# FutureAGI/Xenoverse

Measured on AMD Instinct MI355X. Metric: env-steps/sec (whole node), anymdp |S|=64 |A|=8, 65k envs/GPU, higher is better.
Workload: dtype f64

## Files before the change

### xenoverse_amd/csrc/anymdp.hip

```cpp
#include "anymdp_cutline.h"
#include "philox.h"
#include "xv_common.h"
#include "xv_pipe.h"

#include <cstddef>
#include <cstdlib>
#include <cstring>
#include <mutex>

#define XV_ANYMDP_BLK 7
#define XV_ANYMDP_MAX_CHAINS 16
#ifndef XV_ANYMDP_NT_OUT
#define XV_ANYMDP_NT_OUT 1
#endif

struct AnyMDPArgs {
  const uint4* lines;
  const int32_t* state_map;
  const uint64_t* term_mask;
  const double* s0_cdf;
  const int32_t* s0_ids;
  const int32_t* max_steps;
  const int32_t* env_task;
  const double2* rs_a;
// ... 1406 lines not shown
      __syncthreads();
      if (own) Qs[tid] = qn;
    } else {
      for (int k = tid; k < SA; k += blockDim.x) {
        const int s = k / A, a = k - s * A;
        double qn = 0.0;
        if (!((tm[s >> 6] >> (s & 63)) & 1ull)) {
          const uint32_t r = ((uint32_t)t * S + s) * A + a;
          double prev = 0.0, acc = 0.0, e_r = 0.0;
          for (int j = 0; j < S; ++j) {
            const uint4 e = *anymdp_entry_ptr(P, r, j);
            const double c = xv_u2d(e.x, e.y), p = c - prev;
            prev = c;
            e_r = fma(p, (double)__uint_as_float(e.z), e_r);
            acc = fma(p, Vs[j], acc);
          }
          qn = fma(gamma, acc, e_r);
        }
        const double q = Qs[k];
        d2 += (qn - q) * (qn - q);
        Qs[SA + ((S + 63) & ~63) + blockDim.x + k] = qn;
      }
      __syncthreads();
      for (int k = tid; k < SA; k += blockDim.x) Qs[k] = Qs[SA + ((S + 63) & ~63) + blockDim.x + k];
    }
    red[tid] = d2;
    __syncthreads();
    for (int w = blockDim.x >> 1; w > 0; w >>= 1) {
      if (tid < w) red[tid] += red[tid + w];
      __syncthreads();
    }
    const double diff = sqrt(red[0] / (double)SA);
    __syncthreads();
    if (diff <= tol) { ++it; break; }
  }
  if (q_out) for (int k = tid; k < SA; k += blockDim.x) q_out[(size_t)t * SA + k] = Qs[k];
  if (greedy_out) {
    for (int j = tid; j < S; j += blockDim.x) {
      int best = 0;
      double v = Qs[j * A];
      for (int a = 1; a < A; ++a) if (Qs[j * A + a] > v) { v = Qs[j * A + a]; best = a; }
      greedy_out[(size_t)t * S + j] = (uint8_t)best;
    }
  }
  if (iters_out && tid == 0) iters_out[t] = it;
}

static inline void anymdp_bind_rng(xv_anymdp* h, uint64_t ticks, bool advance = true) {
  h->a.seed = h->eng->seed;
  h->a.gid_base = h->eng->env_id_base;
  const XvTickBind b = xv_engine_bind_tick(h->eng, ticks, advance);
  h->a.tick = b.tick;
  h->a.tick_dev = b.tick_dev;
}

#define XV_ANYMDP_AUTO_FALLBACKS_CACHED 0.2
#define XV_ANYMDP_AUTO_FALLBACKS_HBM 0.5
static inline double anymdp_auto_fallback_limit(const xv_anymdp* h) {
  const double fence_bytes = (double)h->a.n_task * h->a.S * h->a.A * 128.0;
  return fence_bytes <= 128.0 * 1048576.0 ? XV_ANYMDP_AUTO_FALLBACKS_CACHED : XV_ANYMDP_AUTO_FALLBACKS_HBM;
}
static inline int anymdp_effective_search(const xv_anymdp* h) {
  if (h->search == XV_ANYMDP_SEARCH_BINARY || !h->fast) return XV_ANYMDP_SEARCH_BINARY;
  if (h->a.bucket != nullptr &&
      (h->search == XV_ANYMDP_SEARCH_BUCKET || (h->search == XV_ANYMDP_SEARCH_AUTO && h->census.auto_uses_bucket)))
    return XV_ANYMDP_SEARCH_BUCKET;
  return XV_ANYMDP_SEARCH_FENCE;
}

#ifndef XV_KERNELS_ONLY
static void anymdp_pipe_clear(xv_anymdp* h) {
  h->overlap = 0; h->pipe_failed = false; h->pipe_used_last = false; h->side = nullptr; h->side_for = nullptr;
  memset(&h->gate, 0, sizeof(h->gate));
  h->side_ev[0] = h->side_ev[1] = nullptr;
  h->pgraph[0] = h->pgraph[1] = nullptr; h->pgraph_exec[0] = h->pgraph_exec[1] = nullptr;
  h->tgraph[0] = h->tgraph[1] = nullptr; h->tgraph_exec[0] = h->tgraph_exec[1] = nullptr;
  memset(&h->tpipe_key, 0, sizeof(h->tpipe_key));
  h->d_ptick = nullptr; h->ptick_value = 0; h->ptick_valid = false;
  h->d_snap = nullptr; h->d_snap_w = nullptr; h->fell_seen = 0;
  h->backoff.fell_known = 0; h->backoff.left = 0; h->backoff.len = 32;
  h->backoff_mixed.fell_known = 0; h->backoff_mixed.left = 0; h->backoff_mixed.len = 0;
  memset(&h->pipe_key, 0, sizeof(h->pipe_key));
}
static XvPipeLanes anymdp_pipe_lanes(xv_anymdp* h, bool tokens, int D = 0) {
  XvPipeLanes L;
  L.D = D; L.main = h->eng->stream; L.side_for = &h->side_for; L.fork = &h->side_ev[0];
  L.side[0] = &h->side; L.join[0] = &h->side_ev[1];
  for (int q = 0; q < 2; ++q) {
    L.graph[q] = tokens ? &h->tgraph[q] : &h->pgraph[q];
    L.exec[q] = tokens ? &h->tgraph_exec[q] : &h->pgraph_exec[q];
  }
  for (int i = 0; i < XV_PIPE_DEPTH_MAX - 2; ++i) {
    XvPipeDeepLanes& X = h->gate.deep;
    L.side[1 + i] = &X.side[i]; L.join[1 + i] = &X.join[i]; L.graph[2 + i] = &X.graph[i]; L.exec[2 + i] = &X.exec[i];
  }
  return L;
}
static void anymdp_pipe_drop_graphs(xv_anymdp* h) {
  xv_pipe_drop_set(anymdp_pipe_lanes(h, false));
  xv_pipe_drop_set(anymdp_pipe_lanes(h, true));
  memset(&h->pipe_key, 0, sizeof(h->pipe_key));
  memset(&h->tpipe_key, 0, sizeof(h->tpipe_key));
  h->gate.unroll[0] = h->gate.unroll[1] = 0;
  h->gate.depth = 0;
  h->ptick_valid = false;
}
static void anymdp_pipe_release(xv_anymdp* h) {
  anymdp_pipe_drop_graphs(h);
  xv_pipe_release_streams(anymdp_pipe_lanes(h, false));
  if (h->d_ptick) (void)hipFree(h->d_ptick);
  if (h->d_snap) (void)hipFree(h->d_snap);
  if (h->d_snap_w) (void)hipFree(h->d_snap_w);
  xv_pipe_gate_destroy(&h->gate);
  anymdp_pipe_clear(h);
}

extern "C" int xv_anymdp_create(xv_engine* e, int n_env, int n_task, int S, int A, int s0_max,
                                void* rows, const int32_t* state_map, const uint64_t* term_mask,
                                const double* s0_cdf, const int32_t* s0_ids, const int32_t* max_steps,
                                const int32_t* env_task, xv_anymdp** out) {
  XV_CHECK_ARG(out != nullptr);
  *out = nullptr;
  XV_CHECK_ARG(e != nullptr);
  XV_CHECK_ARG(n_env > 0 && n_task > 0);
  XV_CHECK_ARG(S >= 2 && S <= 512 && A >= 2 && A <= 64 && s0_max >= 1 && s0_max <= 256);
  XV_CHECK_ARG(rows && state_map && term_mask && s0_cdf && s0_ids && max_steps && env_task);
  const int NB0 = (S + XV_ANYMDP_BLK - 1) / XV_ANYMDP_BLK, G = (NB0 + 15) / 16;
  const int NB = (NB0 + G - 1) / G * G, RL = 1 + NB;
  XV_CHECK_ARG((uint64_t)n_task * S * A * RL < 0xFFFFFFFFull);
  XV_HIP(hipSetDevice(e->device));
  xv_anymdp* h = new (std::nothrow) xv_anymdp();
  if (!h) {
    xv_set_error("xv_anymdp_create: out of host memory");
    return XV_ERR_NOMEM;
  }
  h->eng = e;
  h->search = XV_ANYMDP_SEARCH_AUTO;
  h->fast = false;
  h->obs_cdf = nullptr; h->n_obs = 0; h->d_obs = 0; h->d_act = 0; h->obs_bucket = nullptr;
  h->max_obs = -1;
  memset(&h->census, 0, sizeof(h->census));
  h->graph_mode = 2; h->graph_failed = false; h->graph = nullptr; h->graph_exec = nullptr;
  h->d_tick = nullptr; h->d_tick_value = 0; h->d_tick_valid = false;
  memset(&h->graph_key, 0, sizeof(h->graph_key));
  h->parent = nullptr; h->view_lo = 0; h->n_views = 0; h->chain_ev = nullptr;
  h->cgraph = nullptr; h->cgraph_exec = nullptr;
  memset(&h->cgraph_key, 0, sizeof(h->cgraph_key));
  anymdp_pipe_clear(h);
  AnyMDPArgs& a = h->a;
  memset(&a, 0, sizeof(a));
  a.lines = (const uint4*)rows; a.state_map = state_map; a.term_mask = term_mask;
  a.s0_cdf = s0_cdf; a.s0_ids = s0_ids; a.max_steps = max_steps; a.env_task = env_task;
  a.n_env = n_env; a.n_task = n_task; a.S = S; a.A = A; a.s0_max = s0_max; a.words = (S + 63) / 64;
  a.NB = NB; a.RL = RL; a.G = G;
  a.err = e->d_err;
  a.seed = e->seed; a.gid_base = e->env_id_base; a.tick = 0;

  bool fast = (G <= 5 && s0_max <= 4);
  auto device_max = [&](const int32_t* p, size_t n, int* out_max) -> hipError_t {
    int* d_max = nullptr;
    hipError_t r = hipMalloc(&d_max, sizeof(int));
    if (r == hipSuccess) r = hipMemsetAsync(d_max, 0, sizeof(int), e->stream);
    if (r == hipSuccess) {
      hipLaunchKernelGGL(anymdp_max_obs_kernel, dim3((unsigned)((n + 255) / 256)), dim3(256), 0, e->stream, p, n, d_max);
      r = hipMemcpyAsync(out_max, d_max, sizeof(int), hipMemcpyDeviceToHost, e->stream);
    }
    if (r == hipSuccess) r = hipStreamSynchronize(e->stream);
    if (d_max) (void)hipFree(d_max);
    return r;
  };
  {
    int h_max = 0;
    hipError_t r = hipSuccess;
    if (fast) {
      r = device_max(state_map, (size_t)n_task * S, &h_max);
      fast = r == hipSuccess && h_max < 65536;
      if (r == hipSuccess) h->max_obs = h_max;
    }
    if (fast) {
      r = device_max(max_steps, (size_t)n_task, &h_max);
      fast = r == hipSuccess && h_max < (1 << 27);
    }
    if (r != hipSuccess) {
// ... 572 lines not shown
```

### xenoverse_amd/csrc/anymdp_many.h

```cpp
#pragma once

struct AnyMDPRings {
  size_t stride;
  const int32_t* actions; int32_t* obs; float* reward; float* reward_gt; uint8_t* terminated; uint8_t* truncated; int32_t* final_obs;
  AnyMDPStepIO slot(int j) const {
    const size_t o = (size_t)j * stride;
    return anymdp_io(actions + o, obs + o, reward + o, reward_gt + o, terminated + o, truncated + o, final_obs ? final_obs + o : nullptr);
  }
  AnyMDPRings shifted(size_t lo) const {
    return AnyMDPRings{stride, actions + lo, obs + lo, reward + lo, reward_gt + lo, terminated + lo, truncated + lo,
                       final_obs ? final_obs + lo : nullptr};
  }
};

struct AnyMDPTokRings {
  const int32_t* actions; int32_t* obs; float* reward; float* reward_gt; uint8_t* terminated; uint8_t* truncated; int32_t* final_obs;
  AnyMDPTokIO slot(const xv_anymdp* h, int j) const {
    const size_t o = (size_t)j * (size_t)h->a.n_env, da = (size_t)h->d_act, dob = (size_t)h->d_obs;
    return anymdp_tok_io(actions + o * da, obs + o * dob, reward + o, reward_gt + o, terminated + o, truncated + o,
                         final_obs ? final_obs + o * dob : nullptr);
  }
};

template <class R> static void anymdp_ring_pointers(const R& r, const void** p) {
// ... 99 lines not shown
  h->d_tick_valid = false;
}

template <class Ensure>
static bool anymdp_many_prepare(xv_anymdp* h, int n_steps, int period, bool wanted, bool sticky, Ensure&& ensure) {
  h->graph_used_last = false;
  if (n_steps / period <= 0 || period <= 1 || h->graph_failed || !wanted) return false;
  bool ok = ensure();
  if (ok && !(h->d_tick_valid && h->d_tick_value == h->eng->tick)) {
    hipLaunchKernelGGL(anymdp_set_tick_kernel, dim3(1), dim3(1), 0, h->eng->stream, h->d_tick, h->eng->tick);
    ok = hipGetLastError() == hipSuccess;
    if (ok) { h->d_tick_value = h->eng->tick; h->d_tick_valid = true; }
  }
  if (!ok) anymdp_many_failed(h, sticky);
  return ok;
}

static bool anymdp_many_cycle(xv_anymdp* h, hipGraphExec_t exec, int period, bool sticky) {
  if (hipGraphLaunch(exec, h->eng->stream) != hipSuccess) {
    anymdp_many_failed(h, sticky);
    return false;
  }
  h->eng->tick += (uint64_t)period;
  h->d_tick_value = h->eng->tick;
  h->d_tick_valid = true;
  h->graph_used_last = true;
  return true;
}

static int anymdp_many_plain(xv_anymdp* h, int k, int period, const AnyMDPRings& R, int mode) {
  anymdp_bind_rng(h, 1);
  return anymdp_launch_step<false>(h, R.slot(k % period), 1, mode);
}

#define XV_ANYMDP_PIPE_GRAPH_MIN 64
static bool anymdp_pipe_setup(xv_anymdp* h, int* D) {
  const XvPipeLanes L = anymdp_pipe_lanes(h, false);
  if (xv_pipe_streams_stale(L)) anymdp_pipe_drop_graphs(h);
  const int got = xv_pipe_ensure_streams(L, *D);
  if (got == 0) return false;
  if (got < *D) (void)hipGetLastError();
  *D = got;
  if (!h->d_ptick && hipMalloc(&h->d_ptick, XV_PIPE_DEPTH_MAX * sizeof(uint64_t)) != hipSuccess) return false;
  if (!h->gate.d_seen && !xv_pipe_gate_create(&h->gate)) return false;
  if (!h->d_snap && hipMalloc(&h->d_snap, (size_t)h->a.n_env * sizeof(uint2)) != hipSuccess) { h->d_snap = nullptr; return false; }
  if (!h->d_snap_w) {
    if (hipMalloc(&h->d_snap_w, 4 * sizeof(uint32_t)) != hipSuccess) { h->d_snap_w = nullptr; return false; }
    if (hipMemsetAsync(h->d_snap_w, 0, 4 * sizeof(uint32_t), h->eng->stream) != hipSuccess) return false;
  }
  return true;
}
static bool anymdp_launch_replay(xv_anymdp* h, int eff, const AnyMDPStepIO& io, int period, int cycles, int mode, uint64_t t0) {
  AnyMDPArgs a = h->a;
  a.seed = h->eng->seed; a.gid_base = h->eng->env_id_base; a.tick = t0; a.tick_dev = nullptr;
  const dim3 grid(xv_div_up(h->a.n_env, 256)), block(256);
  uint32_t* h_fell = h->gate.d_issued + 1;
  anymdp_select_variant(h->a.G, anymdp_variant_bk(h, eff), -1, [&](auto v) {
    using V = decltype(v);
    if constexpr (V::g != 0)
      hipLaunchKernelGGL((anymdp_replay_kernel<V::g, V::bk>), grid, block, 0, h->eng->stream, a, io, period, cycles, mode,
                         (const uint2*)h->d_snap, h->d_snap_w, h->a.err, h_fell);
  });
  return hipGetLastError() == hipSuccess;
}

template <class K, class Node>
static int anymdp_pipe_graph_set(xv_anymdp* h, bool tokens, int D, int period, int cycles, const K& want, K* key, Node&& node,
                                 bool buildable = true) {
  const hipGraphExec_t* exec = tokens ? h->tgraph_exec : h->pgraph_exec;
  const bool same = exec[0] && exec[1] && anymdp_key_same(want, *key);
  const int have = (same && h->gate.depth == D) ? h->gate.unroll[tokens] : 0;
  const int U = xv_pipe_pick_unroll(period, cycles, have, D);
  if (U == 0 || U == have) return U;
  anymdp_pipe_drop_graphs(h);
  if (!buildable || !xv_pipe_build_set(anymdp_pipe_lanes(h, tokens, D), &h->gate, U, period, reinterpret_cast<void*>(&anymdp_pipe_head_kernel),
                                       h->d_ptick, h->a.err, node))
    return -1;
  h->gate.depth = D;
  anymdp_key_store(key, want);
  h->gate.unroll[tokens] = U;
  return U;
}

static int anymdp_pipe_graphs(xv_anymdp* h, int D, int period, int cycles, const AnyMDPRings& R, int mode) {
  const int eff = anymdp_effective_search(h);
  decltype(h->pipe_key) want;
  memset(&want, 0, sizeof want);
  want.period = period; want.mode = mode; want.search = eff; want.stride = R.stride;
  anymdp_ring_pointers(R, want.ptrs);
  want.bucket = (const void*)h->a.bucket; want.seed = h->eng->seed; want.gid_base = h->eng->env_id_base;
  void* fn = anymdp_graph_step_fn(h, eff, mode, true);
  AnyMDPStepNode sn;
  return anymdp_pipe_graph_set(h, false, D, period, cycles, want, &h->pipe_key, [&](int g, int slot, int q, hipKernelNodeParams* np) {
    sn.fill(np, h, fn, h->d_ptick + q, g, slot, R, mode);
  }, fn != nullptr);
}

static __global__ __launch_bounds__(256) void anymdp_pipe_open_kernel(uint2* sr, int n, uint32_t tag, uint64_t* tick_words, int n_words,
                                                                      uint64_t tick_base, uint2* snap, uint32_t* snap_w, uint32_t* err,
                                                                      int bad_tag_env, int repairable) {
  const int i = blockIdx.x * blockDim.x + threadIdx.x;
  if (i < n) {
    uint2 r = sr[i];
    r.x &= (1u << XV_ANYMDP_SR_TAG_SHIFT) - 1u;
    snap[i] = r;
    r.x |= (i == bad_tag_env ? ((tag + 77u) & 0x3FFFu) : tag) << XV_ANYMDP_SR_TAG_SHIFT;
    sr[i] = r;
  }
  if (i < n_words) tick_words[i] = tick_base;
  if (i == 0 && repairable) { const uint32_t e = *err; snap_w[0] = e; snap_w[1] = 0u; snap_w[2] = 0u; *err = e & ~(uint32_t)XV_DEVERR_HANDOFF; }
}

template <class Graphs, class Replay>
static int anymdp_pipe_call(xv_anymdp* h, int n_steps, int ring_period, int min_steps, const void* fn, bool tokens, int32_t* obs,
                            size_t n_obs, int* issued, Graphs&& graphs, Replay&& replay) {
  *issued = 0;
  int D = xv_pipe_preflight(n_steps, ring_period, min_steps, &h->backoff, &h->gate, fn, 256, (size_t)xv_div_up(h->a.n_env, 256),
                            h->eng->device, h->eng->stream);
  if (D == 0) return XV_OK;
  const int U = anymdp_pipe_setup(h, &D) ? graphs(D, n_steps / ring_period) : -1;
  if (U < 0) {
    (void)hipGetLastError();
    h->pipe_failed = true;
    return XV_OK;
  }
  if (U == 0) return XV_OK;
  const int cycles = n_steps / ring_period / U, period = ring_period * U;
  hipStream_t st = h->eng->stream;
  const int test_bad_tag = getenv("XV_PIPE_TEST_BAD_TAG") ? atoi(getenv("XV_PIPE_TEST_BAD_TAG")) : 0;
  const int test_fail = getenv("XV_PIPE_TEST_FAIL") ? atoi(getenv("XV_PIPE_TEST_FAIL")) : 0;
  h->fell_seen = __atomic_load_n(h->gate.h_issued + 1, __ATOMIC_ACQUIRE);
  const uint64_t t0 = h->eng->tick;
  hipLaunchKernelGGL(anymdp_pipe_open_kernel, dim3(xv_div_up(h->a.n_env, 256)), dim3(256), 0, st, h->a.sr, h->a.n_env,
                     XV_ANYMDP_SR_TAG(t0), h->d_ptick, XV_PIPE_DEPTH_MAX, t0 - (uint64_t)period, h->d_snap, h->d_snap_w,
                     h->a.err, test_bad_tag ? 0 : -1, 1);
  const XvPipeLanes L = anymdp_pipe_lanes(h, tokens, h->gate.depth);
  h->ptick_valid = false;
  if (hipGetLastError() != hipSuccess || !xv_pipe_fork(L)) {
    (void)hipGetLastError();
    h->pipe_failed = true;
    return XV_OK;
  }
  const XvPipeIssued r = xv_pipe_issue(L, &h->gate, cycles);
  const int k = r.cycles * period;
  h->eng->tick = t0 + (uint64_t)k;
  if (r.cycles < cycles) { (void)hipGetLastError(); h->pipe_failed = true; }
  *issued = k;
  if (r.broken || !r.joined) {
    (void)hipGetLastError();
    h->pipe_failed = true;
    xv_set_error("xv_anymdp_step_many: an overlapped ring cycle could be issued only in part; the envs' states are undefined");
    return XV_ERR_HIP;
  }
  if (k > 0) {
    if (test_fail)
      hipLaunchKernelGGL(anymdp_test_fail_kernel, dim3(xv_div_up(h->a.n_env, 256)), dim3(256), 0, st, h->a.sr, h->a.n_env, h->a.err, obs, n_obs);
    if (!replay(k, t0)) {
      (void)hipGetLastError();
      h->pipe_failed = true;
    }
    h->ptick_value = h->eng->tick; h->ptick_valid = true; h->graph_used_last = true; h->pipe_used_last = true;
  }
  return XV_OK;
}

static int anymdp_pipe_run(xv_anymdp* h, int n_steps, int period, const AnyMDPRings& R, int mode, int* issued) {
  static const int min_steps = getenv("XV_ANYMDP_PIPE_MIN_STEPS") ? atoi(getenv("XV_ANYMDP_PIPE_MIN_STEPS")) : XV_ANYMDP_PIPE_GRAPH_MIN;
  const int eff = anymdp_effective_search(h);
  return anymdp_pipe_call(h, n_steps, period, min_steps, anymdp_graph_step_fn(h, eff, mode, true), false, R.obs, (size_t)period * (size_t)h->a.n_env,
                          issued, [&](int D, int cycles) { return anymdp_pipe_graphs(h, D, period, cycles, R, mode); },
                          [&](int k, uint64_t t0) { return anymdp_launch_replay(h, eff, R.slot(0), period, k / period, mode, t0); });
}

extern "C" int xv_anymdp_set_step_many_overlap(xv_anymdp* h, int on) {
  XV_CHECK_ARG(h != nullptr && (on == 0 || on == 1));
  const int dev = h->eng->device;
  XV_CHECK_ARG(dev >= 0 && dev < 64);
  if (on) {
    if (h->parent != nullptr) {
      xv_set_error("xv_anymdp_set_step_many_overlap: not on a view (overlap the parent's step_many instead)");
      return XV_ERR_UNSUPPORTED;
    }
    if (!xv_device_overlap_acquire(dev, h)) {
      xv_set_error("xv_anymdp_set_step_many_overlap: another handle on device %d has the overlap on; one at a time", dev);
      return XV_ERR_UNSUPPORTED;
    }
    h->pipe_failed = false;
    xv_pipe_backoff_reset(&h->backoff, &h->gate);
    h->backoff_mixed.len = 0;
  } else {
    xv_device_overlap_release(dev, h);
  }
  h->overlap = on;
  return XV_OK;
}

extern "C" int xv_anymdp_step_many_overlap_state(xv_anymdp* h) {
  if (!h) return 0;
  if (h->pipe_failed) return -1;
  if (h->overlap && h->pipe_used_last && h->gate.h_issued &&
      __atomic_load_n(h->gate.h_issued + 1, __ATOMIC_ACQUIRE) != h->fell_seen)
    return -2;
  return (h->overlap && h->pipe_used_last) ? 1 : 0;
}

extern "C" int xv_anymdp_step_many(xv_anymdp* h, int n_steps, int period, const int32_t* actions,
                                   int32_t* obs, float* reward, float* reward_gt, uint8_t* terminated,
                                   uint8_t* truncated, int32_t* final_obs, int autoreset_mode) {
  XV_CHECK_ARG(h && n_steps > 0 && period > 0);
  XV_CHECK_ARG(actions && obs && reward && reward_gt && terminated && truncated);
  XV_CHECK_ARG(autoreset_mode >= 0 && autoreset_mode <= 2);
  const AnyMDPRings R{(size_t)h->a.n_env, actions, obs, reward, reward_gt, terminated, truncated, final_obs};
  int k = 0;
  const int cycles = n_steps / period;
  h->pipe_used_last = false;
  if (h->overlap && h->graph_mode != 0 && !h->eng->dev_tick && !h->pipe_failed &&
      anymdp_effective_search(h) != XV_ANYMDP_SEARCH_BINARY) {
    XV_HIP(hipSetDevice(h->eng->device));
    h->graph_used_last = false;
    const int rc = anymdp_pipe_run(h, n_steps, period, R, autoreset_mode, &k);
    if (rc != XV_OK) return rc;
  }
  if (k == 0 && anymdp_many_prepare(h, n_steps, period, anymdp_graph_wanted(h, n_steps), true,
                                    [&] { return anymdp_ensure_graph(h, period, R, autoreset_mode); }))
    for (int c = 0; c < cycles && anymdp_many_cycle(h, h->graph_exec, period, true); ++c) k += period;
  for (; k < n_steps; ++k) {
    const int rc = anymdp_many_plain(h, k, period, R, autoreset_mode);
    if (rc != XV_OK) return rc;
  }
  return XV_OK;
}

static bool anymdp_ensure_chain_graph(xv_anymdp* p, xv_anymdp* const* views, int n_views, int period, const AnyMDPRings& R, int mode) {
  const int eff = anymdp_effective_search(p);
  decltype(p->cgraph_key) want;
  memset(&want, 0, sizeof want);
  want.period = period; want.mode = mode; want.search = eff; want.n_views = n_views;
  anymdp_ring_pointers(R, want.ptrs);
  want.bucket = (const void*)p->a.bucket;
  for (int v = 0; v < n_views; ++v) want.views[v] = (const void*)views[v];
  if (p->cgraph_exec && anymdp_key_same(want, p->cgraph_key)) return true;
  anymdp_drop_chain_graph(p);
  if (!p->d_tick && hipMalloc(&p->d_tick, sizeof(uint64_t)) != hipSuccess) return false;
  if (hipGraphCreate(&p->cgraph, 0) != hipSuccess) return false;
  hipGraphNode_t tails[XV_ANYMDP_MAX_CHAINS];
  for (int v = 0; v < n_views; ++v) {
    tails[v] = nullptr;
    if (!anymdp_add_chain(views[v], p->cgraph, &tails[v], p->d_tick, eff, period, R.shifted((size_t)views[v]->view_lo), mode)) return false;
  }
  if (!anymdp_add_tick_node(p->cgraph, tails, n_views, p->d_tick, period)) return false;
  if (hipGraphInstantiate(&p->cgraph_exec, p->cgraph, nullptr, nullptr, 0) != hipSuccess) { p->cgraph_exec = nullptr; return false; }
  anymdp_key_store(&p->cgraph_key, want);
  return true;
// ... 31 lines not shown
  }
  int k = 0;
  if (how == 1) {
    if (anymdp_many_prepare(p, n_steps, period, p->graph_mode != 0, false,
                            [&] { return anymdp_ensure_chain_graph(p, views, n_views, period, R, autoreset_mode); }))
      for (int c = 0; c < cycles && anymdp_many_cycle(p, p->cgraph_exec, period, false); ++c) k += period;
    for (; k < n_steps; ++k) {
      const int rc = anymdp_many_plain(p, k, period, R, autoreset_mode);
      if (rc != XV_OK) return rc;
    }
    for (int v = 0; v < n_views; ++v) views[v]->eng->tick = t0 + (uint64_t)n_steps;
    return XV_OK;
  }
  if (!p->chain_ev) XV_HIP(hipEventCreateWithFlags(&p->chain_ev, hipEventDisableTiming));
  XV_HIP(hipEventRecord(p->chain_ev, p->eng->stream));
  bool all_graph = true;
  for (int v = 0; v < n_views; ++v) {
    xv_anymdp* h = views[v];
    if (h->eng->stream != p->eng->stream) XV_HIP(hipStreamWaitEvent(h->eng->stream, p->chain_ev, 0));
    all_graph = anymdp_many_prepare(h, n_steps, period, h->graph_mode != 0, true,
                                    [&] { return anymdp_ensure_graph(h, period, Rv(v), autoreset_mode); }) && all_graph;
  }
  int rc = XV_OK;
  if (all_graph) {
    for (int c = 0; c < cycles && all_graph; ++c) {
      for (int v = 0; v < n_views; ++v) all_graph = anymdp_many_cycle(views[v], views[v]->graph_exec, period, true) && all_graph;
      if (all_graph) k += period;
    }
    p->graph_used_last = k > 0;
  }
  for (int v = 0; v < n_views; ++v) k = (int)(views[v]->eng->tick - t0) > k ? (int)(views[v]->eng->tick - t0) : k;
  for (int v = 0; v < n_views && rc == XV_OK; ++v)
    for (int kk = (int)(views[v]->eng->tick - t0); kk < k && rc == XV_OK; ++kk)
      rc = anymdp_many_plain(views[v], kk, period, Rv(v), autoreset_mode);
  for (; k < n_steps && rc == XV_OK; ++k)
    for (int v = 0; v < n_views && rc == XV_OK; ++v) rc = anymdp_many_plain(views[v], k, period, Rv(v), autoreset_mode);
  for (int v = 0; v < n_views; ++v) {
    xv_anymdp* h = views[v];
    if (h->eng->stream == p->eng->stream) continue;
    if (!h->chain_ev && hipEventCreateWithFlags(&h->chain_ev, hipEventDisableTiming) != hipSuccess) { rc = rc == XV_OK ? XV_ERR_HIP : rc; continue; }
    if (hipEventRecord(h->chain_ev, h->eng->stream) != hipSuccess ||
        hipStreamWaitEvent(p->eng->stream, h->chain_ev, 0) != hipSuccess)
      rc = rc == XV_OK ? XV_ERR_HIP : rc;
  }
  if (rc == XV_ERR_HIP) xv_set_error("xv_anymdp_step_many_chains: joining the chains failed: %s", hipGetErrorString(hipGetLastError()));
  if (rc == XV_OK) p->eng->tick = t0 + (uint64_t)n_steps;
  return rc;
}

static int anymdp_tok_pipe_graphs(xv_anymdp* h, int D, int period, int cycles, const AnyMDPTokRings& R, int mode) {
  decltype(h->tpipe_key) want;
  memset(&want, 0, sizeof want);
  want.period = period; want.mode = mode; want.fmt = h->a.bfmt; want.d_obs = h->d_obs; want.d_act = h->d_act;
  anymdp_ring_pointers(R, want.ptrs);
  want.bucket = (const void*)h->a.bucket; want.obs_bucket = (const void*)h->obs_bucket;
  want.seed = h->eng->seed; want.gid_base = h->eng->env_id_base;
  void* fn = anymdp_tok_hand_fn(h);
  AnyMDPArgs a;
  AnyMDPTokArgs KA{h->obs_cdf, h->n_obs, h->d_obs, h->d_act, h->obs_bucket};
  AnyMDPTokIO io;
  int md = mode;
  void* params[] = {&a, &KA, &io, &md};
  return anymdp_pipe_graph_set(h, true, D, period, cycles, want, &h->tpipe_key, [&](int g, int slot, int q, hipKernelNodeParams* np) {
    a = h->a;
    a.seed = h->eng->seed; a.gid_base = h->eng->env_id_base;
    a.tick = (uint64_t)g; a.tick_dev = h->d_ptick + q;
    io = R.slot(h, slot);
    np->func = fn; np->gridDim = dim3(xv_div_up(h->a.n_env, 256)); np->blockDim = dim3(256); np->kernelParams = params;
  });
}

extern "C" int xv_anymdp_step_tokens_many(xv_anymdp* h, int n_steps, int period, const int32_t* action, int32_t* obs,
                                          float* reward, float* reward_gt, uint8_t* terminated, uint8_t* truncated,
                                          int32_t* final_obs, int autoreset_mode) {
  XV_CHECK_ARG(h && h->obs_cdf && n_steps > 0 && period > 0);
  XV_CHECK_ARG(action && obs && reward && reward_gt && terminated && truncated);
  XV_CHECK_ARG(autoreset_mode >= 0 && autoreset_mode <= 2);
  const AnyMDPTokRings R{action, obs, reward, reward_gt, terminated, truncated, final_obs};
  int k = 0;
  h->pipe_used_last = false;
  if (h->overlap && !h->eng->dev_tick && !h->pipe_failed && anymdp_tok_coop(h) && hipSetDevice(h->eng->device) == hipSuccess) {
    const int rc = anymdp_pipe_call(h, n_steps, period, XV_ANYMDP_PIPE_GRAPH_MIN, anymdp_tok_hand_fn(h), true, R.obs,
                                    (size_t)period * (size_t)h->a.n_env * (size_t)h->d_obs, &k,
                                    [&](int D, int cycles) { return anymdp_tok_pipe_graphs(h, D, period, cycles, R, autoreset_mode); },
                                    [&](int kk, uint64_t t0) { return anymdp_tok_launch_replay(h, R.slot(h, 0), period, kk, autoreset_mode, t0); });
    if (rc != XV_OK) return rc;
  }
  for (; k < n_steps; ++k) {
    anymdp_bind_rng(h, 1);
    const int rc = anymdp_tok_launch_step<false>(h, R.slot(h, k % period), autoreset_mode);
    if (rc != XV_OK) return rc;
  }
  return XV_OK;
}
```

### xenoverse_amd/csrc/xv_pipe.h

```cpp
#pragma once
#include <hip/hip_runtime.h>
#include <stdint.h>

#include <chrono>
#include <cstdio>
#include <cstdlib>
#include <cstring>
#include <thread>

#include "xv_common.h"
#include "xv_hand.h"

#define XV_PIPE_PING_STEPS 128
#define XV_PIPE_ACCEPT_RATIO 1.5f
#define XV_PIPE_ACCEPT_SLACK_US 1.0f
#define XV_PIPE_MAX_CANDIDATES 6

static __global__ void xv_pipe_ping_kernel(uint32_t* word, uint32_t want, uint32_t* late) {
  const uint64_t t_begin = wall_clock64();
  while (xv_agent_load32(word) != want) {
    if (wall_clock64() - t_begin > 200000ull) {
      atomicOr(late, 1u);
      break;
    }
// ... 18 lines not shown
  uint32_t w[2] = {0u, 1u};
  float ms = 0.0f;
  ok = ok && hipMemcpy(w, d_words, sizeof(w), hipMemcpyDeviceToHost) == hipSuccess && hipEventElapsedTime(&ms, ev[0], ev[1]) == hipSuccess;
  if (!ok) { (void)hipGetLastError(); return -1.0f; }
  if (w[0] != (uint32_t)n || w[1] != 0u) return -1.0f;
  return ms * 1000.0f / (float)n;
}

struct XvPipeCandidate {
  int priority;
  float two_us;
  float one_us;
  int accepted;
};

static bool xv_pipe_pick_side_stream(hipStream_t main, hipStream_t* out, XvPipeCandidate* report, int* n_report,
                                     hipStream_t other = nullptr ) {
  *out = nullptr;
  if (n_report) *n_report = 0;
  uint32_t* d = nullptr;
  hipEvent_t ev[4] = {nullptr, nullptr, nullptr, nullptr};
  if (hipMalloc(&d, 2 * sizeof(uint32_t)) != hipSuccess) { (void)hipGetLastError(); return false; }
  bool ok = true;
  for (int i = 0; i < 4; ++i) ok = ok && hipEventCreate(&ev[i]) == hipSuccess;
  int least = 0, greatest = 0;
  (void)hipDeviceGetStreamPriorityRange(&least, &greatest);
  const int prio[XV_PIPE_MAX_CANDIDATES] = {greatest, 0, 0, least, 0, 0};
  float one = -1.0f;
  if (ok) {
    (void)xv_pipe_pingpong(main, nullptr, d, ev, 16);
    one = xv_pipe_pingpong(main, nullptr, d, ev, XV_PIPE_PING_STEPS);
    const float one_again = xv_pipe_pingpong(main, nullptr, d, ev, XV_PIPE_PING_STEPS);
    if (one_again > 0.0f && (one <= 0.0f || one_again < one)) one = one_again;
    ok = one > 0.0f;
  }
  hipStream_t rejected[XV_PIPE_MAX_CANDIDATES];
  int n_rej = 0;
  for (int c = 0; ok && c < XV_PIPE_MAX_CANDIDATES && !*out; ++c) {
    hipStream_t s = nullptr;
    if (hipStreamCreateWithPriority(&s, hipStreamNonBlocking, prio[c]) != hipSuccess) { (void)hipGetLastError(); continue; }
    (void)xv_pipe_pingpong(main, s, d, ev, 16);
    float two = xv_pipe_pingpong(main, s, d, ev, XV_PIPE_PING_STEPS);
    {
      const float again = xv_pipe_pingpong(main, s, d, ev, XV_PIPE_PING_STEPS);
      if (again > 0.0f && (two <= 0.0f || again < two)) two = again;
    }
    bool take = two > 0.0f && two <= XV_PIPE_ACCEPT_RATIO * one + XV_PIPE_ACCEPT_SLACK_US;
    if (take && other) {
      float pair = xv_pipe_pingpong(other, s, d, ev, XV_PIPE_PING_STEPS);
      const float again = xv_pipe_pingpong(other, s, d, ev, XV_PIPE_PING_STEPS);
      if (again > 0.0f && (pair <= 0.0f || again < pair)) pair = again;
      take = pair > 0.0f && pair <= XV_PIPE_ACCEPT_RATIO * one + XV_PIPE_ACCEPT_SLACK_US;
      if (pair > two || pair <= 0.0f) two = pair;
    }
    if (getenv("XV_PIPE_DEBUG"))
      fprintf(stderr, "xv_pipe: candidate %d priority %d: two streams %.2f us, one stream %.2f us per launch -> %s\n", c, prio[c],
              (double)two, (double)one, take ? "taken" : "rejected");
    if (report && n_report) {
      report[*n_report] = XvPipeCandidate{prio[c], two, one, take ? 1 : 0};
      *n_report += 1;
    }
    if (take) *out = s;
    else rejected[n_rej++] = s;
  }
  for (int i = 0; i < n_rej; ++i) (void)hipStreamDestroy(rejected[i]);
  for (int i = 0; i < 4; ++i) if (ev[i]) (void)hipEventDestroy(ev[i]);
  (void)hipFree(d);
  (void)hipGetLastError();
  return *out != nullptr;
}

#define XV_PIPE_GATE_TIMEOUT 1000000000ull
#define XV_PIPE_GATE_MIN_POLLS (1u << 20)

#define XV_PIPE_DEPTH_MAX 4

struct XvPipeDeepLanes {
  hipStream_t side[XV_PIPE_DEPTH_MAX - 2];
  hipEvent_t join[XV_PIPE_DEPTH_MAX - 2];
  hipGraph_t graph[XV_PIPE_DEPTH_MAX - 2];
  hipGraphExec_t exec[XV_PIPE_DEPTH_MAX - 2];
};

struct XvPipeGate {
  uint32_t* h_issued;
  uint32_t* d_issued;
  uint32_t* d_seen;
  uint32_t issued;
  int unroll[2];
  int depth;
  XvPipeDeepLanes deep;
};

__device__ __forceinline__ void xv_pipe_gate_pass(uint32_t* seen, const uint32_t* issued, uint32_t* err) {
  const uint32_t g = *seen + 1u;
  *seen = g;
  const uint64_t t_begin = wall_clock64();
  uint32_t polls = 0;
  while ((int32_t)(__hip_atomic_load(issued, __ATOMIC_RELAXED, __HIP_MEMORY_SCOPE_SYSTEM) - g) < 0) {
    if (++polls > XV_PIPE_GATE_MIN_POLLS && wall_clock64() - t_begin > XV_PIPE_GATE_TIMEOUT) {
      atomicOr(err, 8u );
      break;
    }
    if ((polls & 63u) == 63u && (xv_agent_load32(err) & 8u)) break;
    __builtin_amdgcn_s_sleep(16);
  }
}

static bool xv_pipe_gate_create(XvPipeGate* g) {
  g->h_issued = nullptr; g->d_issued = nullptr; g->d_seen = nullptr; g->issued = 0; g->unroll[0] = g->unroll[1] = 0; g->depth = 0;
  if (hipHostMalloc(reinterpret_cast<void**>(&g->h_issued), 64, hipHostMallocMapped) != hipSuccess) { g->h_issued = nullptr; return false; }
  for (int i = 0; i < 16; ++i) g->h_issued[i] = 0u;
  if (hipHostGetDevicePointer(reinterpret_cast<void**>(&g->d_issued), g->h_issued, 0) != hipSuccess) return false;
  if (hipMalloc(&g->d_seen, XV_PIPE_DEPTH_MAX * sizeof(uint32_t)) != hipSuccess) { g->d_seen = nullptr; return false; }
  return hipMemset(g->d_seen, 0, XV_PIPE_DEPTH_MAX * sizeof(uint32_t)) == hipSuccess;
}
static bool xv_pipe_gate_sync(XvPipeGate* g) {
  const uint32_t v[XV_PIPE_DEPTH_MAX] = {g->issued, g->issued, g->issued, g->issued};
  return hipMemcpy(g->d_seen, v, sizeof(v), hipMemcpyHostToDevice) == hipSuccess;
}
static void xv_pipe_gate_destroy(XvPipeGate* g) {
  if (g->d_seen) (void)hipFree(g->d_seen);
  if (g->h_issued) (void)hipHostFree(g->h_issued);
  g->h_issued = nullptr; g->d_issued = nullptr; g->d_seen = nullptr; g->issued = 0;
}
static inline void xv_pipe_gate_release(XvPipeGate* g) {
  g->issued += 1u;
  __atomic_store_n(g->h_issued, g->issued, __ATOMIC_RELEASE);
}

static inline void xv_pipe_test_stall(int cycle, int at = 0) {
  if (cycle != 0) return;
  const char* v = getenv("XV_PIPE_TEST_STALL_MS");
  const char* w = getenv("XV_PIPE_TEST_STALL_AT");
  if ((w ? atoi(w) : 0) != at) return;
  if (v && atoi(v) > 0) std::this_thread::sleep_for(std::chrono::milliseconds(atoi(v)));
}

#define XV_PIPE_RESIDENCY_NUM 3
#define XV_PIPE_RESIDENCY_DEN 4
static bool xv_pipe_two_launches_fit(const void* fn, int block_threads, size_t grid_blocks, int device, int n_launches = 2) {
  int per_cu = 0, cus = 0;
  if (hipOccupancyMaxActiveBlocksPerMultiprocessor(&per_cu, fn, block_threads, 0) != hipSuccess ||
      hipDeviceGetAttribute(&cus, hipDeviceAttributeMultiprocessorCount, device) != hipSuccess) {
    (void)hipGetLastError();
    return false;
  }
  if (n_launches > 2 && xv_device_collectives(device) > 0) return false;
  if (n_launches <= 2) return (size_t)n_launches * grid_blocks <= (size_t)per_cu * (size_t)cus;
  return (size_t)n_launches * grid_blocks * XV_PIPE_RESIDENCY_DEN <= (size_t)per_cu * (size_t)cus * XV_PIPE_RESIDENCY_NUM;
}

struct XvPipeBackoff {
  uint32_t fell_known;
  int left;
  int len;
};
static inline void xv_pipe_backoff_reset(XvPipeBackoff* b, const XvPipeGate* g) {
  b->fell_known = g->h_issued ? __atomic_load_n(g->h_issued + 1, __ATOMIC_ACQUIRE) : 0u;
  b->left = 0; b->len = 32;
}
static inline bool xv_pipe_backoff_step(XvPipeBackoff* b, const XvPipeGate* g) {
  if (getenv("XV_PIPE_NO_BACKOFF")) return false;
  if (g->h_issued) {
    const uint32_t fell = __atomic_load_n(g->h_issued + 1, __ATOMIC_ACQUIRE);
    if (fell != b->fell_known) {
      b->fell_known = fell;
      if (b->len < 32) b->len = 32;
      b->left = b->len;
      b->len = b->len >= 2048 ? 4096 : 2 * b->len;
    }
  }
  if (b->left > 0) { --b->left; return true; }
  return false;
}

#define XV_PIPE_GRAPH_STEPS_BIG 128
static inline double xv_pipe_unroll_cost(int period, int cycles, int U, int depth) {
  const int covered = U * (cycles / U) * period, left = cycles * period - covered;
  if (covered <= 0 || (U * period) % depth != 0) return 1.0e30;
  return (double)covered * (1.0 + 1.15 / ((double)U * (double)period / (double)depth)) + 1.3 * (double)left;
}
static inline int xv_pipe_pick_unroll(int period, int cycles, int have, int depth = 2) {
  static const int big_steps = getenv("XV_PIPE_GRAPH_STEPS") ? atoi(getenv("XV_PIPE_GRAPH_STEPS")) : XV_PIPE_GRAPH_STEPS_BIG;
  const int big = (period >= big_steps ? 1 : big_steps / period) * (depth == 2 ? 1 : depth);
  int best = 0;
  double best_cost = 1.0e30;
  for (int U = 1; U <= big && U <= cycles; ++U) {
    const double c = xv_pipe_unroll_cost(period, cycles, U, depth);
    if (c < 1.0e29 && c <= best_cost) { best = U; best_cost = c; }
  }
  if (best == 0) return 0;
  if (have > 0 && have <= cycles && xv_pipe_unroll_cost(period, cycles, have, depth) <= 1.03 * best_cost) return have;
  return best;
}
#define XV_PIPE_DEPTH_DEFAULT 3
static inline int xv_pipe_depth() {
  static const int d = getenv("XV_PIPE_DEPTH") ? atoi(getenv("XV_PIPE_DEPTH")) : XV_PIPE_DEPTH_DEFAULT;
  return d < 2 ? 2 : (d > XV_PIPE_DEPTH_MAX ? XV_PIPE_DEPTH_MAX : d);
}
static int xv_pipe_choose_depth(const void* fn, int block_threads, size_t grid_blocks, int device) {
  for (int d = xv_pipe_depth(); d >= 2; --d)
    if (xv_pipe_two_launches_fit(fn, block_threads, grid_blocks, device, d)) return d;
  return 0;
}

struct XvPipeLanes {
  int D;
  hipStream_t main;
  hipStream_t* side_for;
  hipStream_t* side[XV_PIPE_DEPTH_MAX - 1];
  hipEvent_t* fork;
  hipEvent_t* join[XV_PIPE_DEPTH_MAX - 1];
  hipGraph_t* graph[XV_PIPE_DEPTH_MAX];
  hipGraphExec_t* exec[XV_PIPE_DEPTH_MAX];
  hipStream_t stream(int q) const { return q == 0 ? main : *side[q - 1]; }
};

static inline int xv_pipe_lane_step(int q, int i, int D, int U, int period) {
  const int g = q + i * D;
  return g < U * period ? g : -1;
}
static inline int xv_pipe_step_slot(int g, int period) { return g % period; }

static inline bool xv_pipe_streams_stale(const XvPipeLanes& L) { return *L.side[0] != nullptr && *L.side_for != L.main; }

static hipError_t xv_pipe_drain(const XvPipeLanes& L) {
  hipError_t rc = hipSuccess;
  for (int q = XV_PIPE_DEPTH_MAX - 1; q >= 0; --q) {
    if (q > 0 && !*L.side[q - 1]) continue;
    const hipError_t e = hipStreamSynchronize(L.stream(q));
    if (rc == hipSuccess) rc = e;
  }
  return rc;
}

static void xv_pipe_drop_set(const XvPipeLanes& L) {
  (void)xv_pipe_drain(L);
  for (int q = 0; q < XV_PIPE_DEPTH_MAX; ++q) {
    if (*L.exec[q]) { (void)hipGraphExecDestroy(*L.exec[q]); *L.exec[q] = nullptr; }
    if (*L.graph[q]) { (void)hipGraphDestroy(*L.graph[q]); *L.graph[q] = nullptr; }
  }
}

static void xv_pipe_destroy_streams(const XvPipeLanes& L) {
  for (int i = 0; i < XV_PIPE_DEPTH_MAX - 1; ++i)
    if (*L.side[i]) { (void)hipStreamSynchronize(*L.side[i]); (void)hipStreamDestroy(*L.side[i]); *L.side[i] = nullptr; }
}
static void xv_pipe_release_streams(const XvPipeLanes& L) {
  xv_pipe_destroy_streams(L);
  if (*L.fork) { (void)hipEventDestroy(*L.fork); *L.fork = nullptr; }
  for (int i = 0; i < XV_PIPE_DEPTH_MAX - 1; ++i)
    if (*L.join[i]) { (void)hipEventDestroy(*L.join[i]); *L.join[i] = nullptr; }
}

static int xv_pipe_ensure_streams(const XvPipeLanes& L, int depth) {
  if (xv_pipe_streams_stale(L)) xv_pipe_destroy_streams(L);
  for (int q = 1; q < depth; ++q) {
    hipStream_t* s = L.side[q - 1];
    if (!*s) {
      if (q == 1) *L.side_for = L.main;
      if (!xv_pipe_pick_side_stream(L.main, s, nullptr, nullptr, q == 1 ? nullptr : *L.side[0])) { *s = nullptr; return q == 1 ? 0 : 2; }
    }
    if (q == 1 && !*L.fork && hipEventCreateWithFlags(L.fork, hipEventDisableTiming) != hipSuccess) return 0;
    if (!*L.join[q - 1] && hipEventCreateWithFlags(L.join[q - 1], hipEventDisableTiming) != hipSuccess) return q == 1 ? 0 : 2;
  }
  return depth;
}

static int xv_pipe_preflight(int n_steps, int period, int min_steps, XvPipeBackoff* backoff, const XvPipeGate* gate, const void* fn,
                             int block_threads, size_t grid_blocks, int device, hipStream_t main, int depth_cap = XV_PIPE_DEPTH_MAX) {
  const int cycles = n_steps / period;
  if (cycles <= 0 || period % 2 != 0 || n_steps < min_steps) return 0;
  if (xv_pipe_backoff_step(backoff, gate)) return 0;
  int D = xv_pipe_choose_depth(fn, block_threads, grid_blocks, device);
  if (D > depth_cap) D = depth_cap;
  if (D > period) D = period;
  if (D > 2 && xv_pipe_pick_unroll(period, cycles, 0, D) == 0) D = 2;
  if (D < 2) return 0;
  hipStreamCaptureStatus cs = hipStreamCaptureStatusNone;
  if (hipStreamIsCapturing(main, &cs) != hipSuccess || cs != hipStreamCaptureStatusNone) { (void)hipGetLastError(); return 0; }
  return D;
}

template <class StepFn>
static bool xv_pipe_build_set(const XvPipeLanes& L, XvPipeGate* gate, int U, int period, void* head_fn, uint64_t* tick_words,
                              uint32_t* err, StepFn&& step) {
  if (!xv_pipe_gate_sync(gate)) return false;
  for (int q = 0; q < L.D; ++q) {
    if (hipGraphCreate(L.graph[q], 0) != hipSuccess) return false;
    hipGraphNode_t prev = nullptr;
    {
      uint64_t* t = tick_words + q;
      uint64_t dv = (uint64_t)period * (uint64_t)U;
      uint32_t* seen = gate->d_seen + q;
      const uint32_t* issued = gate->d_issued;
      void* params[] = {&t, &dv, &seen, &issued, &err};
      hipKernelNodeParams np;
      memset(&np, 0, sizeof(np));
      np.func = head_fn; np.gridDim = dim3(1); np.blockDim = dim3(1); np.kernelParams = params;
      if (hipGraphAddKernelNode(&prev, *L.graph[q], nullptr, 0, &np) != hipSuccess) return false;
    }
    for (int i = 0, g; (g = xv_pipe_lane_step(q, i, L.D, U, period)) >= 0; ++i) {
      hipKernelNodeParams np;
      memset(&np, 0, sizeof(np));
      step(g, xv_pipe_step_slot(g, period), q, &np);
      hipGraphNode_t node = nullptr;
      if (hipGraphAddKernelNode(&node, *L.graph[q], &prev, 1, &np) != hipSuccess) return false;
      prev = node;
    }
    if (hipGraphInstantiate(L.exec[q], *L.graph[q], nullptr, nullptr, 0) != hipSuccess) { *L.exec[q] = nullptr; return false; }
  }
  return true;
}

static bool xv_pipe_fork(const XvPipeLanes& L) {
  bool ok = hipEventRecord(*L.fork, L.main) == hipSuccess;
  for (int q = 1; q < L.D; ++q) ok = ok && hipStreamWaitEvent(L.stream(q), *L.fork, 0) == hipSuccess;
  return ok;
}
struct XvPipeIssued {
  int cycles;
  bool broken;
  bool joined;
};
static XvPipeIssued xv_pipe_issue(const XvPipeLanes& L, XvPipeGate* gate, int cycles) {
  XvPipeIssued r{0, false, true};
  for (int c = 0; c < cycles; ++c) {
    if (hipGraphLaunch(*L.exec[0], L.main) != hipSuccess) break;
    for (int q = 1; q < L.D && !r.broken; ++q) {
      if (q <= 2) xv_pipe_test_stall(c, q - 1);
      if (hipGraphLaunch(*L.exec[q], L.stream(q)) != hipSuccess) r.broken = true;
    }
    xv_pipe_gate_release(gate);
    if (r.broken) break;
    r.cycles += 1;
  }
  for (int q = 1; q < L.D; ++q)
    r.joined = hipEventRecord(*L.join[q - 1], L.stream(q)) == hipSuccess && hipStreamWaitEvent(L.main, *L.join[q - 1], 0) == hipSuccess && r.joined;
  return r;
}
```

Measured before the change: 15.94 billion.

## Plan pipelined graph replays as head, unrolled body and tail sets

Replaces the single-unroll graph plan for the non-token anymdp pipeline with a cost-model planner. The planner can add a head graph set and a tail graph set around repeated body replays, so leftover ring cycles that fell back to plain launches get covered by graphs and the first-launch bubble is modelled. It adds extra cached graph sets per lane, a per-call getenv, and new tick offset bookkeeping, which raises graph memory and correctness risk.

```diff
diff --git a/xenoverse_amd/csrc/anymdp.hip b/xenoverse_amd/csrc/anymdp.hip
--- a/xenoverse_amd/csrc/anymdp.hip
+++ b/xenoverse_amd/csrc/anymdp.hip
@@ -1512,7 +1512,7 @@
   h->backoff_mixed.fell_known = 0; h->backoff_mixed.left = 0; h->backoff_mixed.len = 0;
   memset(&h->pipe_key, 0, sizeof(h->pipe_key));
 }
-static XvPipeLanes anymdp_pipe_lanes(xv_anymdp* h, bool tokens, int D = 0) {
+static XvPipeLanes anymdp_pipe_lanes(xv_anymdp* h, bool tokens, int D = 0, int edge = -1) {
   XvPipeLanes L;
   L.D = D; L.main = h->eng->stream; L.side_for = &h->side_for; L.fork = &h->side_ev[0];
   L.side[0] = &h->side; L.join[0] = &h->side_ev[1];
@@ -1524,11 +1524,20 @@
     XvPipeDeepLanes& X = h->gate.deep;
     L.side[1 + i] = &X.side[i]; L.join[1 + i] = &X.join[i]; L.graph[2 + i] = &X.graph[i]; L.exec[2 + i] = &X.exec[i];
   }
+  if (edge >= 0)
+    for (int q = 0; q < XV_PIPE_DEPTH_MAX; ++q) { L.graph[q] = &h->gate.edge[edge].graph[q]; L.exec[q] = &h->gate.edge[edge].exec[q]; }
   return L;
+}
+static void anymdp_pipe_drop_mdp_set(xv_anymdp* h, int edge) {
+  xv_pipe_drop_set(anymdp_pipe_lanes(h, false, 0, edge));
+  if (edge >= 0) h->gate.edge[edge].cycles = 0;
+  else h->gate.unroll[0] = 0;
+  h->ptick_valid = false;
 }
 static void anymdp_pipe_drop_graphs(xv_anymdp* h) {
   xv_pipe_drop_set(anymdp_pipe_lanes(h, false));
   xv_pipe_drop_set(anymdp_pipe_lanes(h, true));
+  for (int e = 0; e < 2; ++e) anymdp_pipe_drop_mdp_set(h, e);
   memset(&h->pipe_key, 0, sizeof(h->pipe_key));
   memset(&h->tpipe_key, 0, sizeof(h->tpipe_key));
   h->gate.unroll[0] = h->gate.unroll[1] = 0;
diff --git a/xenoverse_amd/csrc/anymdp_many.h b/xenoverse_amd/csrc/anymdp_many.h
--- a/xenoverse_amd/csrc/anymdp_many.h
+++ b/xenoverse_amd/csrc/anymdp_many.h
@@ -205,7 +205,7 @@
   return U;
 }
 
-static int anymdp_pipe_graphs(xv_anymdp* h, int D, int period, int cycles, const AnyMDPRings& R, int mode) {
+static int anymdp_pipe_graphs(xv_anymdp* h, int D, int period, int cycles, const AnyMDPRings& R, int mode, XvPipePlan* plan) {
   const int eff = anymdp_effective_search(h);
   decltype(h->pipe_key) want;
   memset(&want, 0, sizeof want);
@@ -213,10 +213,31 @@
   anymdp_ring_pointers(R, want.ptrs);
   want.bucket = (const void*)h->a.bucket; want.seed = h->eng->seed; want.gid_base = h->eng->env_id_base;
   void* fn = anymdp_graph_step_fn(h, eff, mode, true);
+  if (!fn) return -1;
+  if (!anymdp_key_same(want, h->pipe_key) || h->gate.depth != D) anymdp_pipe_drop_graphs(h);
+  const XvPipePlan have{h->gate.edge[0].cycles, h->gate.unroll[0], 0, h->gate.edge[1].cycles};
+  *plan = xv_pipe_plan(period, cycles, D, have, xv_pipe_caps());
+  if (getenv("XV_PIPE_DEBUG"))
+    fprintf(stderr, "xv_pipe: plan for %d ring cycles of %d on %d lanes: head %d, body %d x %d, tail %d\n", cycles, period, D, plan->head,
+            plan->unroll, plan->replays, plan->tail);
+  if (plan->none()) return 0;
+  const int edge[3] = {0, -1, 1}, need[3] = {plan->head, plan->unroll, plan->tail}, built[3] = {have.head, have.unroll, have.tail};
   AnyMDPStepNode sn;
-  return anymdp_pipe_graph_set(h, false, D, period, cycles, want, &h->pipe_key, [&](int g, int slot, int q, hipKernelNodeParams* np) {
-    sn.fill(np, h, fn, h->d_ptick + q, g, slot, R, mode);
-  }, fn != nullptr);
+  for (int i = 0; i < 3; ++i) {
+    if (need[i] == 0 || need[i] == built[i]) continue;
+    anymdp_pipe_drop_mdp_set(h, edge[i]);
+    const int n = need[i] * period;
+    if (!xv_pipe_build_set(anymdp_pipe_lanes(h, false, D, edge[i]), &h->gate, need[i], period, reinterpret_cast<void*>(&anymdp_pipe_head_kernel),
+                           h->d_ptick, h->a.err, [&](int g, int slot, int q, hipKernelNodeParams* np) {
+                             sn.fill(np, h, fn, h->d_ptick + q, g - n, slot, R, mode);
+                           }))
+      return -1;
+    if (edge[i] >= 0) h->gate.edge[edge[i]].cycles = need[i];
+    else h->gate.unroll[0] = need[i];
+    h->gate.depth = D;
+    anymdp_key_store(&h->pipe_key, want);
+  }
+  return 1;
 }
 
 static __global__ __launch_bounds__(256) void anymdp_pipe_open_kernel(uint2* sr, int n, uint32_t tag, uint64_t* tick_words, int n_words,
@@ -241,21 +262,22 @@
   int D = xv_pipe_preflight(n_steps, ring_period, min_steps, &h->backoff, &h->gate, fn, 256, (size_t)xv_div_up(h->a.n_env, 256),
                             h->eng->device, h->eng->stream);
   if (D == 0) return XV_OK;
-  const int U = anymdp_pipe_setup(h, &D) ? graphs(D, n_steps / ring_period) : -1;
-  if (U < 0) {
+  XvPipePlan plan{0, 0, 0, 0};
+  const int got = anymdp_pipe_setup(h, &D) ? graphs(D, n_steps / ring_period, &plan) : -1;
+  if (got < 0) {
     (void)hipGetLastError();
     h->pipe_failed = true;
     return XV_OK;
   }
-  if (U == 0) return XV_OK;
-  const int cycles = n_steps / ring_period / U, period = ring_period * U;
+  if (got == 0 || plan.none()) return XV_OK;
+  const uint64_t words_back = tokens ? (uint64_t)(plan.unroll * ring_period) : 0ull;
   hipStream_t st = h->eng->stream;
   const int test_bad_tag = getenv("XV_PIPE_TEST_BAD_TAG") ? atoi(getenv("XV_PIPE_TEST_BAD_TAG")) : 0;
   const int test_fail = getenv("XV_PIPE_TEST_FAIL") ? atoi(getenv("XV_PIPE_TEST_FAIL")) : 0;
   h->fell_seen = __atomic_load_n(h->gate.h_issued + 1, __ATOMIC_ACQUIRE);
   const uint64_t t0 = h->eng->tick;
   hipLaunchKernelGGL(anymdp_pipe_open_kernel, dim3(xv_div_up(h->a.n_env, 256)), dim3(256), 0, st, h->a.sr, h->a.n_env,
-                     XV_ANYMDP_SR_TAG(t0), h->d_ptick, XV_PIPE_DEPTH_MAX, t0 - (uint64_t)period, h->d_snap, h->d_snap_w,
+                     XV_ANYMDP_SR_TAG(t0), h->d_ptick, XV_PIPE_DEPTH_MAX, t0 - words_back, h->d_snap, h->d_snap_w,
                      h->a.err, test_bad_tag ? 0 : -1, 1);
   const XvPipeLanes L = anymdp_pipe_lanes(h, tokens, h->gate.depth);
   h->ptick_valid = false;
@@ -264,10 +286,23 @@
     h->pipe_failed = true;
     return XV_OK;
   }
-  const XvPipeIssued r = xv_pipe_issue(L, &h->gate, cycles);
-  const int k = r.cycles * period;
+  XvPipeIssued r{0, false, true};
+  int k = 0;
+  {
+    const int kind_edge[3] = {0, -1, 1}, kind_sets[3] = {plan.head > 0 ? 1 : 0, plan.replays, plan.tail > 0 ? 1 : 0};
+    const int kind_cycles[3] = {plan.head, plan.unroll, plan.tail};
+    bool whole = true;
+    for (int i = 0, first = 0; i < 3 && whole; first += kind_sets[i], ++i) {
+      if (kind_sets[i] == 0) continue;
+      const int done = xv_pipe_launch_sets(anymdp_pipe_lanes(h, tokens, h->gate.depth, tokens ? -1 : kind_edge[i]), &h->gate, kind_sets[i], first, &r.broken);
+      r.cycles += done;
+      k += done * kind_cycles[i] * ring_period;
+      whole = done == kind_sets[i];
+    }
+    r.joined = xv_pipe_join(L);
+    if (!whole) { (void)hipGetLastError(); h->pipe_failed = true; }
+  }
   h->eng->tick = t0 + (uint64_t)k;
-  if (r.cycles < cycles) { (void)hipGetLastError(); h->pipe_failed = true; }
   *issued = k;
   if (r.broken || !r.joined) {
     (void)hipGetLastError();
@@ -288,10 +323,11 @@
 }
 
 static int anymdp_pipe_run(xv_anymdp* h, int n_steps, int period, const AnyMDPRings& R, int mode, int* issued) {
-  static const int min_steps = getenv("XV_ANYMDP_PIPE_MIN_STEPS") ? atoi(getenv("XV_ANYMDP_PIPE_MIN_STEPS")) : XV_ANYMDP_PIPE_GRAPH_MIN;
+  const char* ms = getenv("XV_ANYMDP_PIPE_MIN_STEPS");
+  const int min_steps = ms ? atoi(ms) : XV_ANYMDP_PIPE_GRAPH_MIN;
   const int eff = anymdp_effective_search(h);
   return anymdp_pipe_call(h, n_steps, period, min_steps, anymdp_graph_step_fn(h, eff, mode, true), false, R.obs, (size_t)period * (size_t)h->a.n_env,
-                          issued, [&](int D, int cycles) { return anymdp_pipe_graphs(h, D, period, cycles, R, mode); },
+                          issued, [&](int D, int cycles, XvPipePlan* plan) { return anymdp_pipe_graphs(h, D, period, cycles, R, mode, plan); },
                           [&](int k, uint64_t t0) { return anymdp_launch_replay(h, eff, R.slot(0), period, k / period, mode, t0); });
 }
 
@@ -489,7 +525,11 @@
   if (h->overlap && !h->eng->dev_tick && !h->pipe_failed && anymdp_tok_coop(h) && hipSetDevice(h->eng->device) == hipSuccess) {
     const int rc = anymdp_pipe_call(h, n_steps, period, XV_ANYMDP_PIPE_GRAPH_MIN, anymdp_tok_hand_fn(h), true, R.obs,
                                     (size_t)period * (size_t)h->a.n_env * (size_t)h->d_obs, &k,
-                                    [&](int D, int cycles) { return anymdp_tok_pipe_graphs(h, D, period, cycles, R, autoreset_mode); },
+                                    [&](int D, int cycles, XvPipePlan* plan) {
+                                      const int U = anymdp_tok_pipe_graphs(h, D, period, cycles, R, autoreset_mode);
+                                      if (U > 0) *plan = XvPipePlan{0, U, cycles / U, 0};
+                                      return U > 0 ? 1 : U;
+                                    },
                                     [&](int kk, uint64_t t0) { return anymdp_tok_launch_replay(h, R.slot(h, 0), period, kk, autoreset_mode, t0); });
     if (rc != XV_OK) return rc;
   }
diff --git a/xenoverse_amd/csrc/xv_pipe.h b/xenoverse_amd/csrc/xv_pipe.h
--- a/xenoverse_amd/csrc/xv_pipe.h
+++ b/xenoverse_amd/csrc/xv_pipe.h
@@ -124,6 +124,12 @@
   hipGraphExec_t exec[XV_PIPE_DEPTH_MAX - 2];
 };
 
+struct XvPipeEdgeSet {
+  hipGraph_t graph[XV_PIPE_DEPTH_MAX];
+  hipGraphExec_t exec[XV_PIPE_DEPTH_MAX];
+  int cycles;
+};
+
 struct XvPipeGate {
   uint32_t* h_issued;
   uint32_t* d_issued;
@@ -132,6 +138,7 @@
   int unroll[2];
   int depth;
   XvPipeDeepLanes deep;
+  XvPipeEdgeSet edge[2];
 };
 
 __device__ __forceinline__ void xv_pipe_gate_pass(uint32_t* seen, const uint32_t* issued, uint32_t* err) {
@@ -236,6 +243,81 @@
   if (have > 0 && have <= cycles && xv_pipe_unroll_cost(period, cycles, have, depth) <= 1.03 * best_cost) return have;
   return best;
 }
+#define XV_PIPE_SET_COST 1.15
+#define XV_PIPE_PLAIN_RATIO 2.0
+#define XV_PIPE_FIRST_FIXED 5.0
+#define XV_PIPE_NODE_ENQ 0.02
+#define XV_PIPE_HEAD_STEPS 0
+#define XV_PIPE_TAIL_MIN_STEPS 4
+struct XvPipePlan {
+  int head, unroll, replays, tail;
+  int covered() const { return head + unroll * replays + tail; }
+  bool none() const { return covered() == 0; }
+};
+struct XvPipeCaps {
+  int body_steps;
+  int head_steps;
+  int tail_min_steps;
+};
+static inline XvPipeCaps xv_pipe_caps() {
+  const char *b = getenv("XV_PIPE_GRAPH_STEPS"), *h = getenv("XV_PIPE_HEAD_STEPS"), *t = getenv("XV_PIPE_TAIL_MIN_STEPS");
+  XvPipeCaps c{b ? atoi(b) : XV_PIPE_GRAPH_STEPS_BIG, h ? atoi(h) : XV_PIPE_HEAD_STEPS, t ? atoi(t) : XV_PIPE_TAIL_MIN_STEPS};
+  if (c.body_steps < 1) c.body_steps = 1;
+  if (c.head_steps < 0) c.head_steps = 0;
+  if (c.tail_min_steps < 1) c.tail_min_steps = 1;
+  return c;
+}
+static inline int xv_pipe_plan_quantum(int period, int depth) {
+  int m = 1;
+  while ((m * period) % depth != 0) ++m;
+  return m;
+}
+static inline double xv_pipe_plan_cost(int period, int cycles, int depth, const XvPipePlan& p) {
+  if (p.none() || p.covered() > cycles) return 1.0e30;
+  const int sets = (p.head > 0) + p.replays + (p.tail > 0);
+  int first = p.head, second = p.replays > 0 ? p.unroll : p.tail;
+  if (first == 0) { first = second; second = p.replays > 1 ? p.unroll : (p.replays == 1 ? p.tail : 0); }
+  const double D = (double)depth;
+  auto enqueue = [&](int c) { return D * (XV_PIPE_FIRST_FIXED + XV_PIPE_NODE_ENQ * (1.0 + (double)(c * period) / D)); };
+  double bubble = second > 0 ? enqueue(second) - (double)(first * period) : 0.0;
+  if (bubble < 0.0) bubble = 0.0;
+  return enqueue(first) + bubble + (double)(p.covered() * period) + XV_PIPE_SET_COST * D * (double)sets +
+         XV_PIPE_PLAIN_RATIO * (double)((cycles - p.covered()) * period);
+}
+static inline XvPipePlan xv_pipe_plan_with(int cycles, int head, int unroll, int tail) {
+  XvPipePlan p{head <= cycles ? head : 0, unroll, 0, 0};
+  int left = cycles - p.head;
+  const int t = (tail > 0 && tail <= left) ? tail : 0;
+  p.replays = unroll > 0 ? (left - t) / unroll : 0;
+  if (p.replays == 0) p.unroll = 0;
+  left -= p.unroll * p.replays;
+  p.tail = t <= left ? t : 0;
+  return p;
+}
+static inline XvPipePlan xv_pipe_plan(int period, int cycles, int depth, const XvPipePlan& have, const XvPipeCaps& caps) {
+  XvPipePlan best{0, 0, 0, 0};
+  if (cycles <= 0 || depth < 2 || depth > period) return best;
+  const int m = xv_pipe_plan_quantum(period, depth);
+  const int big = (period >= caps.body_steps ? 1 : caps.body_steps / period) * (depth == 2 ? 1 : depth);
+  int h = caps.head_steps / period < cycles ? caps.head_steps / period : cycles;
+  h -= h % m;
+  double best_cost = 1.0e30;
+  for (int U = 0; U <= big && U <= cycles - h; U += m) {
+    const int rest = (cycles - h) - (U > 0 ? U * ((cycles - h) / U) : 0);
+    const bool tail_ok = rest > 0 && rest * period >= caps.tail_min_steps && rest <= big;
+    const XvPipePlan p = xv_pipe_plan_with(cycles, h, U, tail_ok ? rest : 0);
+    const double c = xv_pipe_plan_cost(period, cycles, depth, p);
+    if (c < 1.0e29 && c <= best_cost) { best = p; best_cost = c; }
+  }
+  if (best.none()) return best;
+  if (have.head + have.unroll + have.tail > 0) {
+    const XvPipePlan a = xv_pipe_plan_with(cycles, have.head, have.unroll, have.tail), b = xv_pipe_plan_with(cycles, have.head, have.unroll, 0);
+    if (xv_pipe_plan_cost(period, cycles, depth, a) <= 1.03 * best_cost) return a;
+    if (xv_pipe_plan_cost(period, cycles, depth, b) <= 1.03 * best_cost) return b;
+  }
+  return best;
+}
+
 #define XV_PIPE_DEPTH_DEFAULT 3
 static inline int xv_pipe_depth() {
   static const int d = getenv("XV_PIPE_DEPTH") ? atoi(getenv("XV_PIPE_DEPTH")) : XV_PIPE_DEPTH_DEFAULT;
@@ -366,19 +448,29 @@
   bool broken;
   bool joined;
 };
+static int xv_pipe_launch_sets(const XvPipeLanes& L, XvPipeGate* gate, int cycles, int first, bool* broken) {
+  int done = 0;
+  for (int c = 0; c < cycles; ++c) {
+    if (hipGraphLaunch(*L.exec[0], L.main) != hipSuccess) break;
+    for (int q = 1; q < L.D && !*broken; ++q) {
+      if (q <= 2) xv_pipe_test_stall(first + c, q - 1);
+      if (hipGraphLaunch(*L.exec[q], L.stream(q)) != hipSuccess) *broken = true;
+    }
+    xv_pipe_gate_release(gate);
+    if (*broken) break;
+    done += 1;
+  }
+  return done;
+}
+static bool xv_pipe_join(const XvPipeLanes& L) {
+  bool joined = true;
+  for (int q = 1; q < L.D; ++q)
+    joined = hipEventRecord(*L.join[q - 1], L.stream(q)) == hipSuccess && hipStreamWaitEvent(L.main, *L.join[q - 1], 0) == hipSuccess && joined;
+  return joined;
+}
 static XvPipeIssued xv_pipe_issue(const XvPipeLanes& L, XvPipeGate* gate, int cycles) {
   XvPipeIssued r{0, false, true};
-  for (int c = 0; c < cycles; ++c) {
-    if (hipGraphLaunch(*L.exec[0], L.main) != hipSuccess) break;
-    for (int q = 1; q < L.D && !r.broken; ++q) {
-      if (q <= 2) xv_pipe_test_stall(c, q - 1);
-      if (hipGraphLaunch(*L.exec[q], L.stream(q)) != hipSuccess) r.broken = true;
-    }
-    xv_pipe_gate_release(gate);
-    if (r.broken) break;
-    r.cycles += 1;
-  }
-  for (int q = 1; q < L.D; ++q)
-    r.joined = hipEventRecord(*L.join[q - 1], L.stream(q)) == hipSuccess && hipStreamWaitEvent(L.main, *L.join[q - 1], 0) == hipSuccess && r.joined;
+  r.cycles = xv_pipe_launch_sets(L, gate, cycles, 0, &r.broken);
+  r.joined = xv_pipe_join(L);
   return r;
 }
```

After: 14.59 billion. 0.915x the previous value.
